# jamtrott/spmv-cache-trace

Hardware: AMD Instinct MI355X
Metric: spmv_csr_gflops (higher is better)
Workload: dtype f64

## Files before the change

### spmv-cache-trace_amd/csrc/csr_wavetile.hpp

```cpp
#pragma once

#include "tile_common.hpp"
#include "csr_blocktile.hpp"

namespace spmv {

constexpr int kShiftedMaxLen = 128;

#if defined(SPMV_HIP_EXPERIMENTS) && defined(SPMV_VI_ABLATE)
constexpr int kViAblate = SPMV_VI_ABLATE;
#else
constexpr int kViAblate = 0;
#endif
__device__ __forceinline__ int scalar_load_i32(const int32_t * p)
{
    typedef const int32_t __attribute__((address_space(4))) * const_ptr;
    return *reinterpret_cast<const_ptr>(reinterpret_cast<uintptr_t>(p));
}
}
#include "csr_stenciltile.hpp"
namespace spmv {

template <int QUADS, bool X32, bool VI = false>
__device__ __forceinline__ void tile_products_shifted(
// ... 378 lines not shown
    for (int p0 = 0; p0 < len; p0 += CH) {
#pragma unroll
        for (int i = 0; i < CH; ++i) {
            if (p0 + i < len) {
                const int c = scalar_load_i32(first_row + p0 + i) + first_row_base;
                xv[i] = X32 ? *reinterpret_cast<const v2d_a8 *>(reinterpret_cast<const char *>(x) + ((unsigned) (c + base) << 3))
                            : *reinterpret_cast<const v2d_a8 *>(x + c + base);
            }
        }
#pragma unroll
        for (int i = 0; i < CH; ++i) {
            if (p0 + i < len) {
                const int bi = lead + p0 + i;
                const int dw = scalar_load_i32(reinterpret_cast<const int32_t *>(vit) + (bi >> 2));
                const double val = vtab[(unsigned) (dw >> ((bi & 3) * 8)) & 0x7Fu];
                zA += val * xv[i].x;
                zB += val * xv[i].y;
            }
        }
    }
    if (both) {
        v2d_a8 out = {yv.x + zA, yv.y + zB};
        __builtin_nontemporal_store(out, reinterpret_cast<v2d_a8 *>(y + r0 + base));
        if (PEER) {
#pragma unroll
            for (int k = 0; k < kMaxPeers; ++k)
                if (k < peers.n) {
                    peers.y[k][r0 + base] = out.x;
                    peers.y[k][r0 + base + 1] = out.y;
                }
        }
    } else if (only_second) {
        y_store<PEER, true>(y, peers, r0 + base + 1, yv.y + zB);
    }
}

template <int LPR>
__device__ __forceinline__ double window_row_sum(const double * prod, int s, int e, int part)
{
    double z0 = 0.0, z1 = 0.0, z2 = 0.0, z3 = 0.0;
    int k = s + part;
    for (; k + 3 * LPR < e; k += 4 * LPR) {
        const double a = prod[k], b = prod[k + LPR], c = prod[k + 2 * LPR], d = prod[k + 3 * LPR];
        z0 += a;
        z1 += b;
        z2 += c;
        z3 += d;
    }
    for (; k < e; k += LPR)
        z0 += prod[k];
    return (z0 + z1) + (z2 + z3);
}

template <int TILE, int QUADS, bool C16, bool X32, bool VI, typename YStore>
__device__ __forceinline__ void tile_rows_multi_window(
    double * prod, const int32_t * __restrict__ p, const int32_t * __restrict__ j, const uint16_t * __restrict__ j16,
    const double * __restrict__ a, const double * __restrict__ x, const double * y_in, int r0, int k0, int k1, int nrows, int meta,
    int cbase, int cols, int lane, const uint8_t * __restrict__ vidx, ValueLookup vtab, YStore && store)
{
    const int kb = k0 & ~3;
    const int lanes_log2 = (meta >> kTileMetaLanesShift) & 0x7;
    const int sub = lane >> lanes_log2, part = lane & ((1 << lanes_log2) - 1);
    const int rowi = sub < nrows ? sub : nrows - 1;
    int ps, pe;
    if (meta & kTileMetaUniform) {
        ps = k0 + rowi * (meta & 0xFFFF);
// ... 6 lines not shown
    const bool narrow = C16 && (meta & kTileMetaNarrow);
    double z = 0.0;
    for (int base = kb; base < k1; base += TILE) {
        const int left = k1 - base;
        const int last = ((left < TILE ? left : TILE) - 1) & ~3;
        if (narrow)
            tile_products_narrow<QUADS, 0, VI>(prod, j16 + base, a + base, x + cbase, (unsigned) (cols - 1 - cbase), last, lane, vidx + base, vtab);
        else
            tile_products_wide<QUADS, X32, VI>(prod, j + base, a + base, x, last, lane, vidx + base, vtab);
        __builtin_amdgcn_fence(__ATOMIC_RELEASE, "wavefront");
        __builtin_amdgcn_wave_barrier();
        __builtin_amdgcn_fence(__ATOMIC_ACQUIRE, "wavefront");
        const int s = (ps > base ? ps : base) - base;
        const int e = (pe < base + TILE ? pe : base + TILE) - base;
        switch (lanes_log2) {
        case 3: z += window_row_sum<8>(prod, s, e, part); break;
        case 4: z += window_row_sum<16>(prod, s, e, part); break;
        default: z += window_row_sum<32>(prod, s, e, part); break;
        }
        __builtin_amdgcn_fence(__ATOMIC_RELEASE, "wavefront");
        __builtin_amdgcn_wave_barrier();
        __builtin_amdgcn_fence(__ATOMIC_ACQUIRE, "wavefront");
    }
    switch (lanes_log2) {
    case 3: z = group_sum<8>(z); break;
    case 4: z = group_sum<16>(z); break;
    case 5: z = group_sum<32>(z); break;
    default: z = group_sum<64>(z); break;
    }
    if (sub < nrows && part == 0)
        store(r0 + sub, yv + z);
}

template <int TILE, bool C16, bool X32, bool XCD, int ABL = 0, int XW = 0, bool PANELS = false, bool VI = false, bool PEER = false, bool LIST = false>
__global__ __launch_bounds__(256, (TILE <= 512 ? 8 : 4)) void csr_wavetile_kernel(
    int ntiles, const int4 * __restrict__ desc, const int32_t * __restrict__ p,
    const int32_t * __restrict__ j, const uint16_t * __restrict__ j16,
    const double * __restrict__ a, const double * __restrict__ x, const double * y_in_arg, double * y_arg,
    int nnz_total, int cols, int exact_order_and_nt, const int32_t * __restrict__ patterns, PanelInfo pinfo,
    const uint8_t * __restrict__ vidx = nullptr, const double * __restrict__ vtable = nullptr, int nvalues = 0,
    PeerY peers = PeerY{}, const int32_t * __restrict__ tile_list = nullptr)
{
    static_assert(!LIST || (!PANELS && !VI && !XCD), "the tile list is for the plain variants that follow a window kernel");
    static_assert(!PEER || !PANELS, "column panels add partial sums atomically: nothing to forward");
    constexpr int QUADS = TILE / 256;
    const int exact_order = exact_order_and_nt & 1;
    const bool nt_y = (exact_order_and_nt & 2) != 0;
    const int group_rows = (exact_order_and_nt >> 8) & 15;
    __shared__ __attribute__((aligned(16))) double prod_all[4][TILE + 4];
    __shared__ __attribute__((aligned(16))) uint32_t first_row_all[C16 ? 4 : 1][C16 ? kShiftedMaxLen : 1];
    __shared__ double vtab_lds[VI ? kMaxIndexedValues : 1];

    const int wave = __builtin_amdgcn_readfirstlane((int) threadIdx.x >> 6);
    const int lane = (int) __lane_id();
    int w;
    double * y = y_arg;
    const double * y_in = y_in_arg;
    if (PANELS) {
        const int pk = (int) blockIdx.x & 7;
        w = pinfo.first[pk] + ((int) blockIdx.x >> 3) * 4 + wave;
        if (w >= pinfo.first[pk + 1])
            return;
        y = y_arg - (size_t) pk * (size_t) pinfo.rows;
    } else {
        w = (XCD ? xcd_remap(blockIdx.x, (ntiles + 3) >> 2, true) : (int) blockIdx.x) * 4 + wave;
        if (!VI && w >= ntiles)
            return;
        if (LIST)
            w = __builtin_amdgcn_readfirstlane(tile_list[w]);
    }
    double * prod = prod_all[wave];
    static_assert(XW == 0 || TILE + 4 - XW >= 256 * (QUADS - 1), "the window may only overlap the last quad's product slots");
    double * xwin = prod + (XW ? TILE + 4 - XW : 0);

    const int wd = VI ? (w < ntiles ? w : ntiles - 1) : w;
    const TilePair dp = load_tile_pair(desc, wd);
    const int4 d0 = dp.d0, d1 = dp.d1;
    ValueLookup vtab{vtab_lds, false, 0.0, 0.0};
    if (VI) {
        vtab.tiny = nvalues <= 2;
        if (vtab.tiny) {
            vtab.t0 = vtable[0];
            vtab.t1 = vtable[1];
        } else {
            if (threadIdx.x < kMaxIndexedValues)
                vtab_lds[threadIdx.x] = vtable[threadIdx.x];
            __syncthreads();
        }
        if (w >= ntiles)
            return;
    }
    const int r0 = __builtin_amdgcn_readfirstlane(d0.x & ~kTileFlagPartial);
    const int partial = __builtin_amdgcn_readfirstlane(d0.x & kTileFlagPartial);
    const int k0 = __builtin_amdgcn_readfirstlane(d0.y);
    const int meta = __builtin_amdgcn_readfirstlane(d0.z);
    if (C16 && (meta & kTileMetaBlockWin))
        return;
    const int maxlen = meta & 0xFFFF;
    const int lanes_log2 = (meta >> kTileMetaLanesShift) & 0x7;
    const int cbase = __builtin_amdgcn_readfirstlane(d0.w);
    const int r1 = __builtin_amdgcn_readfirstlane(d1.x & ~kTileFlagPartial);
    const int k1 = __builtin_amdgcn_readfirstlane(d1.y);
    const int nrows = r1 - r0;
    const int kb = k0 & ~3;

    if (meta & kTileMetaFast) {
        if (VI && !kViAblate && C16 && TILE == 512 && !PANELS && (meta & kTileMetaValueRows) && (meta & kTileMetaShifted) && (meta & kTileMetaUniform)
            && (maxlen <= kLanePerRowMaxLen ? (lanes_log2 == 0 && nrows >= 2) : nrows >= kConstantRowMinRows)) {
            const bool pattern = (meta & kTileMetaPattern) != 0;
            tile_rows_pairs_constant<X32, PEER>(pattern ? patterns + (size_t) cbase * kPatStride + kPatRel : j + k0, pattern ? r0 : 0,
                                                vidx + kb, vtab, x, y_in, y, peers, r0, lane, maxlen, k0 - kb, nrows);
            return;
        }
        if (C16 && TILE == 512 && !PANELS && is_masked_stencil_tile(meta)) {
            const double * yin_t = y_in + r0;
            const double yA = yin_t[lane < nrows ? lane : nrows - 1];
            const double yB = yin_t[lane + kWave < nrows ? lane + kWave : nrows - 1];
            const int32_t * pat = patterns + (size_t) cbase * kPatStride;
            double zA, zB;
            tile_rows_masked_stencil<QUADS, X32, VI && !kViAblate>(prod, pat + kPatRel, __builtin_amdgcn_readfirstlane(pat[0]), j16 + k0, a + kb, vidx + kb,
                                                                   vtab, x, cols, r0, (k1 - 1 - kb) & ~3, lane, k0 - kb, nrows, zA, zB);
            if (lane < nrows)
                y_store<PEER, false>(y, peers, r0 + lane, yA + zA, nt_y);
            if (lane + kWave < nrows)
                y_store<PEER, false>(y, peers, r0 + lane + kWave, yB + zB, nt_y);
            return;
        }
        if (TILE == 512 && !PANELS && nrows > 1 && k1 - kb > TILE && lanes_log2 == 6) {
            const bool narrow = C16 && (meta & kTileMetaNarrow);
            tile_rows_long_registers<X32>(p, j, j16, narrow, a, x, narrow ? cbase : 0, (unsigned) (cols - 1 - (narrow ? cbase : 0)), y_in, r0, k0, k1,
                                          nrows, lane, [&](int idx, double v) { y_store<PEER, false>(y, peers, idx, v, nt_y); });
            return;
        }
        if (TILE == 512 && !PANELS && nrows > 1 && k1 - kb > TILE) {
            tile_rows_multi_window<TILE, QUADS, C16, X32, VI>(prod, p, j, j16, a, x, y_in, r0, k0, k1, nrows, meta, cbase, cols, lane, vidx, vtab,
                                                              [&](int idx, double v) { y_store<PEER, false>(y, peers, idx, v, nt_y); });
            return;
        }
// ... 199 lines not shown
```

### spmv-cache-trace_amd/csrc/internal.hpp

```cpp
#pragma once

#include "spmv_hip_plan.h"
#include "spmv_hip_symmetric.h"
#include "spmv_hip_multivec.h"
#include "spmv_hip_transpose.h"
#include "spmv_hip_f32values.h"
#include "spmv_hip_compact.h"
#include "spmv_hip_compact_f64.h"
#include "spmv_hip_compact_f32xy.h"
#include "spmv_hip_scaled.h"
#include "spmv_hip_dots.h"

#include <hip/hip_runtime.h>
#include <rccl/rccl.h>

#include <atomic>
#include <cstdint>
#include <string>
#include <vector>

#include "spmv_kernels.hpp"
#include "csr_segwin.hpp"

namespace spmvi {
// ... 93 lines not shown
    int split_rows = 0;
    bool balanced = false;
    int32_t * d_colh = nullptr;
    int32_t * d_hub_column = nullptr;
    double * d_hubx = nullptr;
    int nhubs = 0, hub_threshold = 0;
    long long hub_entries = 0;
    int multi_window_tiles = 0;
    int block_hint = 0;
    int block_offset = 0;
    bool block_skewed = false;
    int hints_tried = 0;
    bool hint_from_bits = false;
    int colshare_tiles = 0;
    long long colshare_entries = 0;
    int block_candidate = 0;
    const uint32_t * group_bits = nullptr;
    int block_cuts = 0;
    int break_rows = 0;
    int block_tiles = 0;
    long long block_entries = 0;
    int stencil_mask_tiles = 0;
    long long stencil_mask_entries = 0;
    int masked_block_tiles = 0;
    long long masked_block_entries = 0;
    size_t meta_bytes = 0;
    long long streamed_bytes = 0, shifted_entries = 0, narrow_entries = 0, uniform_rows = 0;
    uint8_t * d_vidx = nullptr;
    double * d_vtab = nullptr;
    int nvalues = 0;
    int value_row_tiles = 0;
    int4 * d_tiles_vi = nullptr;
    int ntiles_vi = 0;
    const double * values_from = nullptr;
    const double * values_wanted = nullptr;
    unsigned long long value_checksum = 0;
    mutable std::atomic<bool> verify_values_pending{false};
    unsigned long long column_checksum = 0;
    mutable std::atomic<bool> verify_pending{false};
};

struct spmv_hip_ctx {
    int device = 0;
    unsigned flags = 0;
    hipStream_t stream = nullptr;
    hipStream_t own_stream = nullptr;
    hipEvent_t ev0 = nullptr, ev1 = nullptr;
    bool timed = false;
    int format = 0;
    int32_t rows = 0, cols = 0, nnz = 0, row_length = 0, nnz2 = 0;
    int csr_algorithm = SPMV_HIP_CSR_AUTO;
    int csr_lanes = 0;
    spmv_hip_plan * plan = nullptr;
    spmv_hip_sym_plan * sym_plan = nullptr;
    spmv_hip_tr_plan * tr_plan = nullptr;
    spmv_hip_f32_plan * f32_plan = nullptr;
    float * d_val32 = nullptr;
    spmv_hip_c16_plan * c16_plan = nullptr;
    float *d_x32 = nullptr, *d_y32 = nullptr;
    double * d_dots = nullptr;
    size_t dots_work_bytes = 0;
    bool dots_run = false;
    spmv_hip_mv_plan * mv_plan = nullptr;
    double *d_bx = nullptr, *d_by = nullptr;
    int block_k = 0;
    bool block_x_set = false;
// ... 81 lines not shown
```

### spmv-cache-trace_amd/csrc/launch.hip

```cpp
#include "internal.hpp"
#ifdef SPMV_HIP_EXPERIMENTS
#include "csr_pipe.hpp"
#include <cstdlib>
#endif

#include <algorithm>

using namespace spmvi;

namespace {

template <bool DENSE, bool NT>
static auto run_kernel(bool yin_nt, bool yout_nt) -> decltype(&spmv::csr_runs_kernel<DENSE, NT, true, true>)
{
    return yin_nt ? (yout_nt ? spmv::csr_runs_kernel<DENSE, NT, true, true> : spmv::csr_runs_kernel<DENSE, NT, true, false>)
                  : (yout_nt ? spmv::csr_runs_kernel<DENSE, NT, false, true> : spmv::csr_runs_kernel<DENSE, NT, false, false>);
}

template <int LPR>
void launch_vector(const spmv_hip_plan * pl, const int32_t * p, const int32_t * j, const double * a,
                   const double * x, double * y, hipStream_t s)
{
    hipLaunchKernelGGL((spmv::csr_vector_kernel<LPR, kBlock>), dim3(pl->workgroups), dim3(kBlock), 0, s,
                       pl->rows, p, j, a, x, y);
// ... 248 lines not shown
                if (peers && pl->split_rows == 0 && !pl->d_blocks && !pl->d_segblocks) {
                    hipLaunchKernelGGL((spmv::csr_wavetile_kernel<512, true, true, false, 0, 256, false, false, true>), dim3(pl->workgroups), dim3(256), 0, s,
                                       pl->ntiles, pl->d_tiles, p, j, pl->d_col16, a, x, y_in, y, pl->nnz, pl->cols, exact, pl->d_patterns, spmv::PanelInfo{},
                                       (const uint8_t *) nullptr, (const double *) nullptr, 0, *peers);
                    *fused = 1;
                } else
                    hipLaunchKernelGGL((spmv::csr_wavetile_kernel<512, true, true, false, 0, 256>), dim3(pl->workgroups), dim3(256), 0, s,
                                       pl->ntiles, pl->d_tiles, p, j, pl->d_col16, a, x, y_in, y, pl->nnz, pl->cols, exact, pl->d_patterns, spmv::PanelInfo{});
            }
#ifdef SPMV_HIP_EXPERIMENTS
            else if (abl && c16 && x32 && pl->tile == 512) {
                if (abl == 1) hipLaunchKernelGGL((spmv::csr_wavetile_kernel<512, true, true, false, 1>), dim3(pl->workgroups), dim3(256), 0, s, pl->ntiles, pl->d_tiles, p, j, pl->d_col16, a, x, y_in, y, pl->nnz, pl->cols, exact, pl->d_patterns, spmv::PanelInfo{});
                else if (abl == 2) hipLaunchKernelGGL((spmv::csr_wavetile_kernel<512, true, true, false, 2>), dim3(pl->workgroups), dim3(256), 0, s, pl->ntiles, pl->d_tiles, p, j, pl->d_col16, a, x, y_in, y, pl->nnz, pl->cols, exact, pl->d_patterns, spmv::PanelInfo{});
                else hipLaunchKernelGGL((spmv::csr_wavetile_kernel<512, true, true, false, 3>), dim3(pl->workgroups), dim3(256), 0, s, pl->ntiles, pl->d_tiles, p, j, pl->d_col16, a, x, y_in, y, pl->nnz, pl->cols, exact, pl->d_patterns, spmv::PanelInfo{});
            }
#endif
            else if (pl->tile == 1024) {
                if (xcd) SPMV_WT_C(1024, true); else SPMV_WT_C(1024, false);
            } else if (peers && c16 && x32 && !xcd && pl->split_rows == 0 && !pl->d_blocks && !pl->d_segblocks) {
                if (pl->nvalues > 0 && pl->values_from == a)
                    hipLaunchKernelGGL((spmv::csr_wavetile_kernel<512, true, true, false, 0, 0, false, true, true>), dim3(vi_groups), dim3(256), 0, s,
                                       vi_ntiles, vi_tiles, p, j, pl->d_col16, a, x, y_in, y, pl->nnz, pl->cols, exact, pl->d_patterns,
                                       spmv::PanelInfo{}, pl->d_vidx, pl->d_vtab, pl->nvalues, *peers);
                else
                    hipLaunchKernelGGL((spmv::csr_wavetile_kernel<512, true, true, false, 0, 0, false, false, true>), dim3(pl->workgroups), dim3(256), 0, s,
                                       pl->ntiles, pl->d_tiles, p, j, pl->d_col16, a, x, y_in, y, pl->nnz, pl->cols, exact, pl->d_patterns,
                                       spmv::PanelInfo{}, (const uint8_t *) nullptr, (const double *) nullptr, 0, *peers);
                *fused = 1;
            } else if (c16 && x32 && pl->nvalues > 0 && pl->values_from == a) {
                if (xcd)
                    hipLaunchKernelGGL((spmv::csr_wavetile_kernel<512, true, true, true, 0, 0, false, true>), dim3(vi_groups), dim3(256), 0, s,
                                       vi_ntiles, vi_tiles, p, j, pl->d_col16, a, x, y_in, y, pl->nnz, pl->cols, exact, pl->d_patterns,
                                       spmv::PanelInfo{}, pl->d_vidx, pl->d_vtab, pl->nvalues);
                else
                    hipLaunchKernelGGL((spmv::csr_wavetile_kernel<512, true, true, false, 0, 0, false, true>), dim3(vi_groups), dim3(256), 0, s,
                                       vi_ntiles, vi_tiles, p, j, pl->d_col16, a, x, y_in, y, pl->nnz, pl->cols, exact, pl->d_patterns,
                                       spmv::PanelInfo{}, pl->d_vidx, pl->d_vtab, pl->nvalues);
            } else {
                if (xcd) SPMV_WT_C(512, true); else SPMV_WT_C(512, false);
            }
#undef SPMV_WT_C
#undef SPMV_WT_X
#undef SPMV_WT_LAUNCH
            if (c16 && pl->d_segblocks) {
                if (rest_forwards) {
                    if (pl->segwin_slots <= 2688)
                        hipLaunchKernelGGL((spmv::csr_segwin_kernel<512, 2688, true>), dim3(pl->nsegblocks), dim3(512), 0, s, pl->d_tiles,
                                           pl->d_segblocks, p, pl->d_col16, a, x, y_in, y, *peers);
                    else
                        hipLaunchKernelGGL((spmv::csr_segwin_kernel<512, 4096, true>), dim3(pl->nsegblocks), dim3(512), 0, s, pl->d_tiles,
                                           pl->d_segblocks, p, pl->d_col16, a, x, y_in, y, *peers);
                    *fused = 1;
                } else if (pl->segwin_slots <= 2688)
                    hipLaunchKernelGGL((spmv::csr_segwin_kernel<512, 2688>), dim3(pl->nsegblocks), dim3(512), 0, s, pl->d_tiles,
                                       pl->d_segblocks, p, pl->d_col16, a, x, y_in, y);
                else
                    hipLaunchKernelGGL((spmv::csr_segwin_kernel<512, 4096>), dim3(pl->nsegblocks), dim3(512), 0, s, pl->d_tiles,
                                       pl->d_segblocks, p, pl->d_col16, a, x, y_in, y);
            } else if (c16 && pl->d_blocks) {
#ifdef SPMV_HIP_EXPERIMENTS
                if (pl->flags & 0x2000u) {
                    hipLaunchKernelGGL((spmv::csr_blockwin_kernel<512>), dim3(pl->nblocks16), dim3(1024), 0, s, pl->ntiles,
                                       pl->d_tiles, pl->d_blocks, p, pl->d_col16, a, x, y_in, y);
                } else
#endif
                {
// ... 140 lines not shown
```

### spmv-cache-trace_amd/csrc/plan_csr.hip

```cpp
#include "internal.hpp"

#include <algorithm>
#include <cstdlib>
#include <cstring>
#include <new>
#include <system_error>
#include <thread>
#include <unordered_map>
#include <utility>

using namespace spmvi;

namespace {

constexpr size_t kStripedInts = (size_t) spmv::kCountStripes * spmv::kCountWidth;

template <typename T>
hipError_t read_striped(const T * d_counters, T * out, int n, hipStream_t s)
{
    T host[kStripedInts];
    hipError_t e = hipMemcpyAsync(host, d_counters, sizeof(host), hipMemcpyDeviceToHost, s);
    if (e == hipSuccess)
        e = hipStreamSynchronize(s);
    for (int i = 0; i < n; ++i) {
// ... 1870 lines not shown
    if (e == hipSuccess && rc == SPMV_HIP_OK) {
        rc = plan_csr_internal(&pl->inner, (int32_t) vrows, pl->cols, vrow_ptr.data(), SPMV_HIP_CSR_WAVETILE, 0,
                               (pl->flags | SPMV_HIP_FLAG_NO_X_WINDOW | SPMV_HIP_FLAG_NO_COLUMN_PANELS) & ~SPMV_HIP_FLAG_ROWS128, rows);
        if (rc == SPMV_HIP_OK)
            rc = spmv_hip_plan_csr_compress(pl->inner, pl->d_pcol, stream);
    }
    if (e != hipSuccess || rc != SPMV_HIP_OK) {
        if (pl->inner) { spmv_hip_plan_destroy(pl->inner); pl->inner = nullptr; }
        if (pl->d_vrow_ptr) { (void) hipFree(pl->d_vrow_ptr); pl->d_vrow_ptr = nullptr; }
        if (pl->d_pcol) { (void) hipFree(pl->d_pcol); pl->d_pcol = nullptr; }
        if (pl->d_pval) { (void) hipFree(pl->d_pval); pl->d_pval = nullptr; }
        return e != hipSuccess ? fail_hip(e, "column panels") : rc;
    }
    pl->pinfo = pl->inner->pinfo;
    int most = 0;
    for (int k = 0; k < 8; ++k)
        most = std::max(most, pl->pinfo.first[k + 1] - pl->pinfo.first[k]);
    pl->panel_blocks = (most + 3) / 4;
    pl->panels_from_col = d_column_index;
    pl->panels_from_val = d_value;
    pl->meta_bytes += (size_t) (vrows + 1) * sizeof(int32_t) + (size_t) pl->nnz * 12 + pl->inner->meta_bytes;
    {
        long long nonempty = 0;
        for (long long v = 0; v < vrows; ++v)
            nonempty += vrow_ptr[(size_t) v + 1] > vrow_ptr[(size_t) v];
        pl->streamed_bytes = pl->inner->streamed_bytes - 16LL * vrows + 16LL * nonempty;
        pl->shifted_entries = pl->inner->shifted_entries;
        pl->narrow_entries = pl->inner->narrow_entries;
        pl->uniform_rows = 0;
    }
    return SPMV_HIP_OK;
}

static hipError_t merge_constant_row_tiles(spmv_hip_plan * pl, const uint8_t * d_same_prev, hipStream_t s)
{
#if defined(SPMV_HIP_EXPERIMENTS) && defined(SPMV_VI_ABLATE)
    return hipSuccess;
#endif
    std::vector<int4> d((size_t) pl->ntiles + 1);
    hipError_t e = read_back(d.data(), pl->d_tiles, d.size() * sizeof(int4), s);
    if (e != hipSuccess)
        return e;
    std::vector<uint8_t> same_prev((size_t) pl->ntiles, 0);
    e = read_back(same_prev.data(), d_same_prev, same_prev.size(), s);
    if (e != hipSuccess)
        return e;
    std::vector<int32_t> pat;
    if (pl->d_patterns && pl->npatterns > 0) {
        pat.resize((size_t) pl->npatterns * spmv::kPatStride);
        e = read_back(pat.data(), pl->d_patterns, pat.size() * sizeof(int32_t), s);
        if (e != hipSuccess)
            return e;
    }
    const int want = spmv::kTileMetaValueRows | spmv::kTileMetaPattern | spmv::kTileMetaFast | spmv::kTileMetaUniform | spmv::kTileMetaShifted;
    auto mergeable = [&](int w) {
        return !(d[(size_t) w].x & spmv::kTileFlagPartial) && (d[(size_t) w].z & want) == want && d[(size_t) w].w >= 0
            && d[(size_t) w].w < pl->npatterns;
    };
    auto same_stencil = [&](int a, int b) {
        const int len = d[(size_t) a].z & 0xFFFF;
        if (len != (d[(size_t) b].z & 0xFFFF))
            return false;
        const int32_t * pa = pat.data() + (size_t) d[(size_t) a].w * spmv::kPatStride + spmv::kPatRel;
        const int32_t * pb = pat.data() + (size_t) d[(size_t) b].w * spmv::kPatStride + spmv::kPatRel;
        return d[(size_t) a].w == d[(size_t) b].w || std::equal(pa, pa + len, pb);
    };
    std::vector<int4> out;
    out.reserve(d.size());
    int merged_runs = 0;
    for (int w = 0; w < pl->ntiles;) {
        if (!mergeable(w)) {
            out.push_back(d[(size_t) w++]);
            continue;
        }
        int e_run = w + 1;
        while (e_run < pl->ntiles && mergeable(e_run) && same_stencil(w, e_run) && same_prev[(size_t) e_run])
            ++e_run;
        const int len = d[(size_t) w].z & 0xFFFF;
        const long long r_begin = d[(size_t) w].x, r_end = d[(size_t) e_run].x & 0x7FFFFFFF, k_begin = d[(size_t) w].y;
        if (e_run - w < 2 || (long long) d[(size_t) e_run].y - k_begin != (r_end - r_begin) * len) {
            for (; w < e_run; ++w)
                out.push_back(d[(size_t) w]);
            continue;
        }
        ++merged_runs;
        const long long run_rows = r_end - r_begin;
        const long long n = (run_rows + 127) / 128;
        if (len > spmv::kLanePerRowMaxLen && run_rows / n < spmv::kConstantRowMinRows) {
            --merged_runs;
            for (; w < e_run; ++w)
                out.push_back(d[(size_t) w]);
            continue;
        }
        long long r = r_begin;
        for (long long i = 0; i < n; ++i) {
            out.push_back(make_int4((int) r, (int) (k_begin + (r - r_begin) * len), d[(size_t) w].z, d[(size_t) w].w));
            r += run_rows / n + (i < run_rows % n ? 1 : 0);
        }
        w = e_run;
    }
    if (merged_runs == 0 || out.size() >= (size_t) pl->ntiles)
        return hipSuccess;
    const int n = (int) out.size();
    out.push_back(d[(size_t) pl->ntiles]);
    e = hipMalloc((void **) &pl->d_tiles_vi, out.size() * sizeof(int4));
    if (e == hipSuccess)
        e = hipMemcpy(pl->d_tiles_vi, out.data(), out.size() * sizeof(int4), hipMemcpyHostToDevice);
    if (e != hipSuccess) {
        if (pl->d_tiles_vi) (void) hipFree(pl->d_tiles_vi);
        pl->d_tiles_vi = nullptr;
        return e;
    }
    pl->ntiles_vi = n;
    return hipSuccess;
}

static void drop_value_dictionary(spmv_hip_plan * pl)
{
    if (pl->d_vidx) (void) hipFree(pl->d_vidx);
    if (pl->d_vtab) (void) hipFree(pl->d_vtab);
    if (pl->d_tiles_vi) (void) hipFree(pl->d_tiles_vi);
    pl->d_vidx = nullptr;
    pl->d_vtab = nullptr;
    pl->d_tiles_vi = nullptr;
    pl->ntiles_vi = 0;
    pl->nvalues = 0;
    pl->values_from = nullptr;
    pl->verify_values_pending = false;
}

int spmv_hip_plan_csr_index_values(spmv_hip_plan * pl, const double * d_value, void * stream)
{
    if (!pl)
        return fail(SPMV_HIP_ERR_INVALID, "plan is null");
    hipStream_t s = static_cast<hipStream_t>(stream);
    const size_t before = (pl->d_vidx ? (size_t) pl->nnz + 64 + spmv::kMaxIndexedValues * sizeof(double) : 0);
    drop_value_dictionary(pl);
    pl->values_wanted = d_value;
    pl->meta_bytes -= std::min(pl->meta_bytes, before);
    const bool other_variant = pl->inner || pl->d_blocks || pl->d_segblocks;
    if (pl->algorithm != SPMV_HIP_CSR_WAVETILE || pl->tile != 512 || pl->nnz == 0 || pl->ntiles == 0
        || (pl->balanced && (pl->flags & SPMV_HIP_FLAG_XCD_REMAP))
        || !pl->d_col16 || other_variant || pl->cols >= (1 << 29)
        || (pl->flags & SPMV_HIP_FLAG_NO_VALUE_INDEX))
        return (pl->inner || before == 0) ? SPMV_HIP_OK
                                          : plan_account(pl, pl->d_col16 != nullptr, s);
    if (!d_value)
        return fail(SPMV_HIP_ERR_INVALID, "null device pointer");
    unsigned long long * d_keys = nullptr;
    int * d_state = nullptr;
    std::vector<unsigned long long> keys((size_t) spmv::kDictSlots, spmv::kDictEmpty);
    int state[2] = {0, 0};
    hipError_t e = hipMalloc((void **) &d_keys, keys.size() * sizeof(unsigned long long));
    if (e == hipSuccess) e = hipMalloc((void **) &d_state, sizeof(state));
    if (e == hipSuccess) e = hipMemcpyAsync(d_keys, keys.data(), keys.size() * sizeof(unsigned long long), hipMemcpyHostToDevice, s);
    if (e == hipSuccess) e = hipMemsetAsync(d_state, 0, sizeof(state), s);
    if (e == hipSuccess && pl->nnz > 16384) {
        hipLaunchKernelGGL(spmv::value_dict_insert_kernel, dim3(1), dim3(256), 0, s, 8192LL, d_value, d_keys, d_state, spmv::kMaxIndexedValues);
// ... 22 lines not shown
        unsigned long long * d_table = nullptr;
        e = hipMalloc((void **) &d_table, (size_t) spmv::kMaxIndexedValues * sizeof(unsigned long long));
        if (e == hipSuccess) e = hipMalloc((void **) &pl->d_vtab, (size_t) spmv::kMaxIndexedValues * sizeof(double));
        if (e == hipSuccess) e = hipMalloc((void **) &pl->d_vidx, (size_t) pl->nnz + 64);
        if (e == hipSuccess) e = hipMemsetAsync(pl->d_vidx, 0, (size_t) pl->nnz + 64, s);
        if (e == hipSuccess) e = hipMemcpyAsync(d_table, table.data(), table.size() * sizeof(unsigned long long), hipMemcpyHostToDevice, s);
        if (e == hipSuccess) e = hipMemcpyAsync(pl->d_vtab, values.data(), values.size() * sizeof(double), hipMemcpyHostToDevice, s);
        if (e == hipSuccess) e = hipMemsetAsync(d_state, 0, sizeof(state), s);
        if (e == hipSuccess) {
            hipLaunchKernelGGL(spmv::value_index_kernel, dim3((unsigned) grid_for(pl->nnz, kBlock, cu_count() * 16)), dim3(256), 0, s,
                               (long long) pl->nnz, d_value, d_table, (int) table.size(), pl->d_vidx, d_state);
            e = hipGetLastError();
        }
        if (e == hipSuccess) e = hipMemcpyAsync(state, d_state, sizeof(state), hipMemcpyDeviceToHost, s);
        if (e == hipSuccess) e = hipStreamSynchronize(s);
        if (d_table) (void) hipFree(d_table);
        pl->value_row_tiles = 0;
        if (e == hipSuccess && state[1] == 0) {
            unsigned long long * d_count = nullptr;
            uint8_t * d_same_prev = nullptr;
            unsigned long long count[2] = {0, 0};
            e = hipMalloc((void **) &d_count, kStripedInts * sizeof(unsigned long long));
            if (e == hipSuccess) e = hipMalloc((void **) &d_same_prev, (size_t) pl->ntiles);
            if (e == hipSuccess) e = hipMemsetAsync(d_count, 0, kStripedInts * sizeof(unsigned long long), s);
            if (e == hipSuccess) {
                hipLaunchKernelGGL(spmv::value_rows_mark_kernel, dim3((unsigned) ((pl->ntiles + 3) / 4)), dim3(256), 0, s, pl->ntiles, pl->d_tiles,
                                   pl->d_vidx, spmv::kConstantRowMaxLen, d_count, d_same_prev);
                e = hipGetLastError();
            }
            if (e == hipSuccess) e = read_striped(d_count, count, 2, s);
            if (d_count) (void) hipFree(d_count);
            pl->value_row_tiles = (int) count[0];
            if (e == hipSuccess && count[0] > 0)
                e = merge_constant_row_tiles(pl, d_same_prev, s);
            if (d_same_prev) (void) hipFree(d_same_prev);
        }
        if (e == hipSuccess && state[1] == 0) {
            pl->nvalues = (int) table.size();
            pl->values_from = d_value;
            rc = device_value_checksum(d_value, pl->nnz, &pl->value_checksum, s);
            pl->verify_values_pending = true;
            pl->meta_bytes += (size_t) pl->nnz + 64 + spmv::kMaxIndexedValues * sizeof(double);
        } else {
            drop_value_dictionary(pl);
        }
    }
    if (d_keys) (void) hipFree(d_keys);
    if (d_state) (void) hipFree(d_state);
    if (e != hipSuccess) {
        drop_value_dictionary(pl);
        return fail_hip(e, "value dictionary");
    }
    if (rc != SPMV_HIP_OK) {
        drop_value_dictionary(pl);
        return rc;
    }
    if (pl->nvalues == 0 && before == 0)
        return SPMV_HIP_OK;
    return plan_account(pl, pl->d_col16 != nullptr, s);
}

int spmv_hip_plan_csr_refresh_values(spmv_hip_plan * pl, const int32_t * d_row_ptr, const int32_t * d_column_index,
                                     const double * d_value, void * stream)
{
    if (!pl)
        return fail(SPMV_HIP_ERR_INVALID, "plan is null");
    if (pl->nvalues > 0 || pl->d_vidx) {
        int rc = spmv_hip_plan_csr_index_values(pl, d_value, stream);
        if (rc != SPMV_HIP_OK)
            return rc;
    }
    if (!pl->inner)
        return SPMV_HIP_OK;
    if (!d_row_ptr || !d_column_index || !d_value)
        return fail(SPMV_HIP_ERR_INVALID, "null device pointer");
    if (d_column_index != pl->panels_from_col)
        return fail(SPMV_HIP_ERR_STATE, "the column panels were made from another column array");
    hipStream_t s = static_cast<hipStream_t>(stream);
    const unsigned grid = (unsigned) ((pl->rows + 255) / 256);
    hipLaunchKernelGGL(spmv::csr_panel_scatter_kernel, dim3(grid), dim3(256), 0, s, pl->rows, (pl->cols + 7) / 8, d_row_ptr,
                       d_column_index, d_value, pl->d_vrow_ptr, pl->d_pcol, pl->d_pval);
    HIP_TRY(hipGetLastError());
    pl->panels_from_val = d_value;
    return SPMV_HIP_OK;
}

int spmv_hip_plan_info(const spmv_hip_plan * pl, int64_t * out, int n)
{
    if (!pl || !out || n < 0)
        return fail(SPMV_HIP_ERR_INVALID, "plan/out null");
    const int64_t v[44] = {pl->algorithm, pl->lanes_per_row, pl->workgroups, pl->nblk,
                           pl->long_blocks, pl->rows, pl->nnz, (int64_t) pl->meta_bytes, pl->narrow_tiles,
                           pl->uniform_tiles, pl->shifted_tiles, pl->xwin_tiles, pl->blockwin_tiles,
                           pl->inner ? pl->inner->ntiles : 0, pl->streamed_bytes, pl->shifted_entries,
                           pl->narrow_entries, pl->uniform_rows, pl->inner ? 1 : 0, pl->balanced ? 1 : 0, pl->nvalues,
                           pl->segwin_tiles, pl->segwin_slots, pl->nvalues > 0 ? pl->value_row_tiles : 0,
                           pl->nvalues > 0 && pl->d_tiles_vi ? pl->ntiles_vi : 0, pl->nvalues > 0 ? 0 : pl->block_tiles,
                           pl->nvalues > 0 ? 0 : pl->block_entries, pl->nhubs, pl->hub_entries, pl->multi_window_tiles,
                           pl->ngroup_tiles, pl->nvalues > 0 ? 0 : pl->masked_block_tiles, pl->nvalues > 0 ? 0 : pl->masked_block_entries,
                           pl->stencil_mask_tiles, pl->stencil_mask_entries,
                           pl->nvalues > 0 ? 0 : pl->colshare_tiles, pl->nvalues > 0 ? 0 : pl->colshare_entries,
                           pl->colshare_tiles > 0 ? pl->block_hint : 0, pl->nrun_chunks, pl->run_tiles, pl->run_entries,
                           pl->run_masked_chunks, pl->nrun_chunks > 0 ? pl->nrun_rest : 0,
                           pl->nrun_chunks > 0 ? 1 + (pl->run_sweep ? 4 : 0) : 0};
    for (int i = 0; i < n && i < 44; ++i)
        out[i] = v[i];
    return SPMV_HIP_OK;
}

}
```

### spmv-cache-trace_amd/python/spmv_amd/capi.py

```python
import ctypes as C
import os

import numpy as np

PKG_ROOT = os.path.dirname(os.path.dirname(os.path.dirname(os.path.abspath(__file__))))
LIB_PATH = os.path.join(PKG_ROOT, "libspmv_hip.so")
EXPERIMENTS_LIB_PATH = os.path.join(PKG_ROOT, "libspmv_hip_experiments.so")
if os.environ.get("SPMV_HIP_EXPERIMENTS") == "1":
    LIB_PATH = EXPERIMENTS_LIB_PATH
elif os.environ.get("SPMV_HIP_EXPERIMENTS", "").endswith(".so"):
    LIB_PATH = os.path.abspath(os.environ["SPMV_HIP_EXPERIMENTS"])
HEADER_PATH = os.path.join(os.path.dirname(PKG_ROOT), "include", "spmv_hip.h")
HEADER_PATHS = [HEADER_PATH] + [os.path.join(os.path.dirname(PKG_ROOT), "include", n)
                                for n in ("spmv_hip_tuning.h", "spmv_hip_plan.h", "spmv_hip_symmetric.h", "spmv_hip_multivec.h",
                                          "spmv_hip_transpose.h", "spmv_hip_f32values.h", "spmv_hip_compact.h",
                                          "spmv_hip_compact_f64.h", "spmv_hip_compact_f32xy.h", "spmv_hip_scaled.h", "spmv_hip_dots.h",
                                          "spmv_hip_krylov.h", "spmv_hip_bicgstab.h", "spmv_hip_gmres.h", "spmv_hip_bjacobi.h",
                                          "spmv_hip_cheby.h", "spmv_hip_mcgs.h")]

OK = 0
ERR_INVALID, ERR_NO_DEVICE, ERR_HIP, ERR_ALLOC, ERR_STATE, ERR_OVERFLOW, ERR_ALIGN = -1, -2, -3, -4, -5, -6, -7
CSR_AUTO, CSR_SCALAR, CSR_VECTOR, CSR_ADAPTIVE, CSR_WAVETILE = 0, 1, 2, 3, 4
FLAG_XCD_REMAP, FLAG_EXACT_ORDER, FLAG_BIG_TILE, FLAG_NO_INDEX_COMPRESSION, FLAG_COO_KEEP_ORDER, FLAG_READ_ROW_PTR, FLAG_ROWS64, FLAG_ROWS128, FLAG_ELL_COLUMN_MAJOR = 0x1, 0x2, 0x8, 0x10, 0x20, 0x40, 0x80, 0x100, 0x200
FLAG_NO_SHIFTED_TILES = 0x400
# ... 451 lines not shown
        check(self.lib.spmv_hip_last_run_times(self.h, C.byref(k), C.byref(g)))
        return k.value, g.value

    def info(self):
        out = np.zeros(20, dtype=np.int64)
        check(self.lib.spmv_hip_ctx_info(self.h, out, 20))
        keys = ["format", "rows", "cols", "stored", "algorithm", "lanes_per_row", "workgroups",
                "row_blocks", "long_blocks", "device_bytes", "narrow_tiles", "shifted_tiles", "xwin_tiles",
                "blockwin_tiles", "panel_tiles", "streamed_bytes", "devices", "ell_path", "rccl_ranks", "pipelined"]
        return dict(zip(keys, out.tolist()))


class CsrPlan:

    def __init__(self, rows, cols, host_row_ptr, algorithm=CSR_AUTO, lanes_per_row=0, flags=0):
        self.lib = load()
        h = _vp()
        check(self.lib.spmv_hip_plan_csr(C.byref(h), rows, cols, _i32(host_row_ptr), algorithm,
                                         lanes_per_row, flags))
        self.h = h

    def close(self):
        if self.h:
            self.lib.spmv_hip_plan_destroy(self.h)
            self.h = None

    def __del__(self):
        try:
            self.close()
        except Exception:
            pass

    def info(self):
        out = np.zeros(44, dtype=np.int64)
        check(self.lib.spmv_hip_plan_info(self.h, out, 44))
        keys = ["algorithm", "lanes_per_row", "workgroups", "row_blocks", "long_blocks", "rows",
                "nnz", "meta_bytes", "narrow_tiles", "uniform_tiles", "shifted_tiles", "xwin_tiles", "blockwin_tiles", "panel_tiles",
                "streamed_bytes", "shifted_entries", "narrow_entries", "uniform_rows", "value_snapshot", "balanced", "indexed_values",
                "segwin_tiles", "segwin_slots", "value_row_tiles", "dictionary_launch_tiles", "block_tiles", "block_entries", "hub_columns", "hub_entries", "multi_window_tiles", "row_group_tiles",
                "masked_block_tiles", "masked_block_entries", "stencil_mask_tiles", "stencil_mask_entries",
                "group_tiles", "group_entries", "group_rows", "run_chunks", "run_tiles", "run_entries",
                "run_masked_chunks", "run_rest_tiles", "run_variant"]
        return dict(zip(keys, out.tolist()))

    def confirm_blocks(self, d_row_ptr, d_col, host_row_ptr=None, stream=0):
        hp = None if host_row_ptr is None else np.ascontiguousarray(host_row_ptr, dtype=np.int32)
        check(self.lib.spmv_hip_plan_csr_confirm_blocks(self.h, d_row_ptr, d_col, None if hp is None else hp.ctypes.data, stream))

    def compress(self, d_col, stream=0):
        check(self.lib.spmv_hip_plan_csr_compress(self.h, d_col, stream))

    def repack(self, d_row_ptr, d_col, d_val, stream=0):
        check(self.lib.spmv_hip_plan_csr_repack(self.h, d_row_ptr, d_col, d_val, stream))

    def spmv(self, d_row_ptr, d_col, d_val, d_x, d_y, stream=0):
        check(self.lib.spmv_hip_csr_spmv(self.h, d_row_ptr, d_col, d_val, d_x, d_y, stream))

    def spmv_out(self, d_row_ptr, d_col, d_val, d_x, d_y_in, d_y_out, stream=0):
        check(self.lib.spmv_hip_csr_spmv_out(self.h, d_row_ptr, d_col, d_val, d_x, d_y_in, d_y_out, stream))

    def verify(self, d_col, stream=0):
        check(self.lib.spmv_hip_plan_verify(self.h, d_col, stream))

    def index_values(self, d_val, stream=0):
        check(self.lib.spmv_hip_plan_csr_index_values(self.h, d_val, stream))

    def refresh_values(self, d_row_ptr, d_col, d_val, stream=0):
        check(self.lib.spmv_hip_plan_csr_refresh_values(self.h, d_row_ptr, d_col, d_val, stream))


def csr_triangle(rows, row_ptr, col):
    row_ptr, col = _i32(row_ptr), _i32(col)
    if len(row_ptr) < rows + 1:
        raise ValueError("row_ptr needs rows + 1 entries")
    if len(col) == 0:
# ... 627 lines not shown
```

Before: 1164.

## Bake dominant constant-value stencil into kernel arguments for value-indexed tiles

During planning, finds the most common (column offset pattern, coefficient) stencil among uniform value-indexed tiles, marks those tiles, and passes the stencil's offsets and coefficients as kernel arguments held in scalar registers. Marked tiles then skip loading column patterns, value indices and the value table and compute each row as a fixed stencil over x, two rows per lane. The plan also re-cuts constant-row runs on 128-row boundaries. This adds a planning pass with a device readback and a new kernel template instance with larger argument pressure, and it only pays off when the matrix has one stencil that dominates.

```diff
diff --git a/spmv-cache-trace_amd/csrc/csr_wavetile.hpp b/spmv-cache-trace_amd/csrc/csr_wavetile.hpp
--- a/spmv-cache-trace_amd/csrc/csr_wavetile.hpp
+++ b/spmv-cache-trace_amd/csrc/csr_wavetile.hpp
@@ -434,6 +434,67 @@
         }
     } else if (only_second) {
         y_store<PEER, true>(y, peers, r0 + base + 1, yv.y + zB);
+    }
+}
+
+constexpr int kDomMaxLen = 8;
+constexpr int kTileMetaDominant = 1 << 21;
+struct DomStencil {
+    int len;
+    int rel[kDomMaxLen];
+    double coef[kDomMaxLen];
+};
+
+template <int LEN, bool TWO>
+__device__ __forceinline__ void tile_rows_dominant(const DomStencil & dom, const double * __restrict__ x, const double * y_in,
+                                                   double * y, int r0, int lane, int nrows)
+{
+    constexpr int P = TWO ? 2 : 1;
+    const int top = nrows - 2;
+    int base[P];
+    v2d_a8 yv[P], xv[P][LEN];
+#pragma unroll
+    for (int q = 0; q < P; ++q)
+        base[q] = 128 * q + 2 * lane < top ? 128 * q + 2 * lane : top;
+#pragma unroll
+    for (int q = 0; q < P; ++q)
+        yv[q] = __builtin_nontemporal_load(reinterpret_cast<const v2d_a8 *>(y_in + r0 + base[q]));
+#pragma unroll
+    for (int q = 0; q < P; ++q)
+#pragma unroll
+        for (int p = 0; p < LEN; ++p)
+            xv[q][p] = *reinterpret_cast<const v2d_a8 *>(reinterpret_cast<const char *>(x) + ((unsigned) (r0 + dom.rel[p] + base[q]) << 3));
+#pragma unroll
+    for (int q = 0; q < P; ++q) {
+        double zA = 0.0, zB = 0.0;
+#pragma unroll
+        for (int p = 0; p < LEN; ++p) {
+            zA += dom.coef[p] * xv[q][p].x;
+            zB += dom.coef[p] * xv[q][p].y;
+        }
+        const int first = 128 * q + 2 * lane;
+        if (first <= top) {
+            const v2d_a8 out = {yv[q].x + zA, yv[q].y + zB};
+            __builtin_nontemporal_store(out, reinterpret_cast<v2d_a8 *>(y + r0 + base[q]));
+        } else if (first == nrows - 1) {
+            __builtin_nontemporal_store(yv[q].y + zB, y + r0 + base[q] + 1);
+        }
+    }
+}
+
+template <bool TWO>
+__device__ __forceinline__ void tile_rows_dominant_any(const DomStencil & dom, const double * __restrict__ x, const double * y_in,
+                                                       double * y, int r0, int lane, int nrows)
+{
+    switch (dom.len) {
+    case 1: tile_rows_dominant<1, TWO>(dom, x, y_in, y, r0, lane, nrows); break;
+    case 2: tile_rows_dominant<2, TWO>(dom, x, y_in, y, r0, lane, nrows); break;
+    case 3: tile_rows_dominant<3, TWO>(dom, x, y_in, y, r0, lane, nrows); break;
+    case 4: tile_rows_dominant<4, TWO>(dom, x, y_in, y, r0, lane, nrows); break;
+    case 5: tile_rows_dominant<5, TWO>(dom, x, y_in, y, r0, lane, nrows); break;
+    case 6: tile_rows_dominant<6, TWO>(dom, x, y_in, y, r0, lane, nrows); break;
+    case 7: tile_rows_dominant<7, TWO>(dom, x, y_in, y, r0, lane, nrows); break;
+    default: tile_rows_dominant<8, TWO>(dom, x, y_in, y, r0, lane, nrows); break;
     }
 }
 
@@ -506,16 +567,18 @@
         store(r0 + sub, yv + z);
 }
 
-template <int TILE, bool C16, bool X32, bool XCD, int ABL = 0, int XW = 0, bool PANELS = false, bool VI = false, bool PEER = false, bool LIST = false>
-__global__ __launch_bounds__(256, (TILE <= 512 ? 8 : 4)) void csr_wavetile_kernel(
+template <int TILE, bool C16, bool X32, bool XCD, int ABL = 0, int XW = 0, bool PANELS = false, bool VI = false, bool PEER = false, bool LIST = false,
+          int DOM = 0>
+__global__ __launch_bounds__(256, (TILE <= 512 ? (DOM == 2 ? 6 : 8) : 4)) void csr_wavetile_kernel(
     int ntiles, const int4 * __restrict__ desc, const int32_t * __restrict__ p,
     const int32_t * __restrict__ j, const uint16_t * __restrict__ j16,
     const double * __restrict__ a, const double * __restrict__ x, const double * y_in_arg, double * y_arg,
     int nnz_total, int cols, int exact_order_and_nt, const int32_t * __restrict__ patterns, PanelInfo pinfo,
     const uint8_t * __restrict__ vidx = nullptr, const double * __restrict__ vtable = nullptr, int nvalues = 0,
-    PeerY peers = PeerY{}, const int32_t * __restrict__ tile_list = nullptr)
+    PeerY peers = PeerY{}, const int32_t * __restrict__ tile_list = nullptr, DomStencil dom = DomStencil{})
 {
     static_assert(!LIST || (!PANELS && !VI && !XCD), "the tile list is for the plain variants that follow a window kernel");
+    static_assert(DOM == 0 || (VI && C16 && X32 && TILE == 512 && !XCD && !PANELS && !PEER && !LIST && ABL == 0 && XW == 0), "the dominant stencil belongs to the default dictionary launch");
     static_assert(!PEER || !PANELS, "column panels add partial sums atomically: nothing to forward");
     constexpr int QUADS = TILE / 256;
     const int exact_order = exact_order_and_nt & 1;
@@ -525,6 +588,10 @@
     __shared__ __attribute__((aligned(16))) uint32_t first_row_all[C16 ? 4 : 1][C16 ? kShiftedMaxLen : 1];
     __shared__ double vtab_lds[VI ? kMaxIndexedValues : 1];
 
+    if (DOM)
+        asm volatile("" ::"s"(x), "s"(y_in_arg), "s"(y_arg), "s"(dom.len), "s"(dom.rel[0]), "s"(dom.rel[1]), "s"(dom.rel[2]), "s"(dom.rel[3]),
+                     "s"(dom.rel[4]), "s"(dom.rel[5]), "s"(dom.rel[6]), "s"(dom.rel[7]), "s"(dom.coef[0]), "s"(dom.coef[1]), "s"(dom.coef[2]),
+                     "s"(dom.coef[3]), "s"(dom.coef[4]), "s"(dom.coef[5]), "s"(dom.coef[6]), "s"(dom.coef[7]));
     const int wave = __builtin_amdgcn_readfirstlane((int) threadIdx.x >> 6);
     const int lane = (int) __lane_id();
     int w;
@@ -578,6 +645,13 @@
     const int nrows = r1 - r0;
     const int kb = k0 & ~3;
 
+    if (DOM && (meta & kTileMetaDominant)) {
+        if (DOM == 2 && nrows > 128)
+            tile_rows_dominant_any<true>(dom, x, y_in, y, r0, lane, nrows);
+        else
+            tile_rows_dominant_any<false>(dom, x, y_in, y, r0, lane, nrows);
+        return;
+    }
     if (meta & kTileMetaFast) {
         if (VI && !kViAblate && C16 && TILE == 512 && !PANELS && (meta & kTileMetaValueRows) && (meta & kTileMetaShifted) && (meta & kTileMetaUniform)
             && (maxlen <= kLanePerRowMaxLen ? (lanes_log2 == 0 && nrows >= 2) : nrows >= kConstantRowMinRows)) {
diff --git a/spmv-cache-trace_amd/csrc/internal.hpp b/spmv-cache-trace_amd/csrc/internal.hpp
--- a/spmv-cache-trace_amd/csrc/internal.hpp
+++ b/spmv-cache-trace_amd/csrc/internal.hpp
@@ -149,6 +149,11 @@
     int value_row_tiles = 0;
     int4 * d_tiles_vi = nullptr;
     int ntiles_vi = 0;
+    bool vi_recut = false;
+    spmv::DomStencil dom_stencil{};
+    int dom_tiles = 0;
+    long long dom_rows = 0;
+    bool dom_two_pairs = false;
     const double * values_from = nullptr;
     const double * values_wanted = nullptr;
     unsigned long long value_checksum = 0;
diff --git a/spmv-cache-trace_amd/csrc/launch.hip b/spmv-cache-trace_amd/csrc/launch.hip
--- a/spmv-cache-trace_amd/csrc/launch.hip
+++ b/spmv-cache-trace_amd/csrc/launch.hip
@@ -304,6 +304,16 @@
                     hipLaunchKernelGGL((spmv::csr_wavetile_kernel<512, true, true, true, 0, 0, false, true>), dim3(vi_groups), dim3(256), 0, s,
                                        vi_ntiles, vi_tiles, p, j, pl->d_col16, a, x, y_in, y, pl->nnz, pl->cols, exact, pl->d_patterns,
                                        spmv::PanelInfo{}, pl->d_vidx, pl->d_vtab, pl->nvalues);
+#ifdef SPMV_HIP_EXPERIMENTS
+                else if (pl->d_tiles_vi && pl->dom_tiles > 0 && pl->dom_two_pairs)
+                    hipLaunchKernelGGL((spmv::csr_wavetile_kernel<512, true, true, false, 0, 0, false, true, false, false, 2>), dim3(vi_groups), dim3(256), 0, s,
+                                       vi_ntiles, vi_tiles, p, j, pl->d_col16, a, x, y_in, y, pl->nnz, pl->cols, exact, pl->d_patterns,
+                                       spmv::PanelInfo{}, pl->d_vidx, pl->d_vtab, pl->nvalues, spmv::PeerY{}, (const int32_t *) nullptr, pl->dom_stencil);
+#endif
+                else if (pl->d_tiles_vi && pl->dom_tiles > 0)
+                    hipLaunchKernelGGL((spmv::csr_wavetile_kernel<512, true, true, false, 0, 0, false, true, false, false, 1>), dim3(vi_groups), dim3(256), 0, s,
+                                       vi_ntiles, vi_tiles, p, j, pl->d_col16, a, x, y_in, y, pl->nnz, pl->cols, exact, pl->d_patterns,
+                                       spmv::PanelInfo{}, pl->d_vidx, pl->d_vtab, pl->nvalues, spmv::PeerY{}, (const int32_t *) nullptr, pl->dom_stencil);
                 else
                     hipLaunchKernelGGL((spmv::csr_wavetile_kernel<512, true, true, false, 0, 0, false, true>), dim3(vi_groups), dim3(256), 0, s,
                                        vi_ntiles, vi_tiles, p, j, pl->d_col16, a, x, y_in, y, pl->nnz, pl->cols, exact, pl->d_patterns,
diff --git a/spmv-cache-trace_amd/csrc/plan_csr.hip b/spmv-cache-trace_amd/csrc/plan_csr.hip
--- a/spmv-cache-trace_amd/csrc/plan_csr.hip
+++ b/spmv-cache-trace_amd/csrc/plan_csr.hip
@@ -1926,10 +1926,116 @@
     return SPMV_HIP_OK;
 }
 
-static hipError_t merge_constant_row_tiles(spmv_hip_plan * pl, const uint8_t * d_same_prev, hipStream_t s)
+static __global__ void first_row_bytes_kernel(int n, const int32_t * __restrict__ k, const uint8_t * __restrict__ vidx,
+                                              unsigned long long * __restrict__ out)
+{
+    const int i = (int) (blockIdx.x * blockDim.x + threadIdx.x);
+    if (i >= n)
+        return;
+    const uint8_t * b = vidx + k[i];
+    unsigned long long v = 0;
+    for (int q = 0; q < 8; ++q)
+        v |= (unsigned long long) b[q] << (8 * q);
+    out[i] = v;
+}
+
+static hipError_t mark_dominant_tiles(spmv_hip_plan * pl, std::vector<int4> & out, int n, const std::vector<int32_t> & pat,
+                                      const std::vector<double> & values, int max_rows, hipStream_t s)
+{
+    pl->dom_stencil = spmv::DomStencil{};
+    pl->dom_tiles = 0;
+    pl->dom_rows = 0;
+    const int want = spmv::kTileMetaValueRows | spmv::kTileMetaPattern | spmv::kTileMetaFast | spmv::kTileMetaUniform | spmv::kTileMetaShifted;
+    std::vector<int> cand;
+    std::vector<int32_t> first;
+    for (int w = 0; w < n; ++w) {
+        const int4 t = out[(size_t) w];
+        const int len = t.z & 0xFFFF, rows = (out[(size_t) w + 1].x & 0x7FFFFFFF) - (t.x & 0x7FFFFFFF);
+        if ((t.x & spmv::kTileFlagPartial) || (t.z & want) != want || (t.z & spmv::kTileMetaBlockWin) || ((t.z >> spmv::kTileMetaLanesShift) & 7) != 0
+            || len < 1 || len > spmv::kDomMaxLen || rows < 2 || rows > max_rows || t.w < 0 || t.w >= pl->npatterns
+            || (long long) out[(size_t) w + 1].y - t.y != (long long) rows * len)
+            continue;
+        cand.push_back(w);
+        first.push_back(t.y);
+    }
+    if (cand.empty())
+        return hipSuccess;
+    std::vector<unsigned long long> bytes(cand.size());
+    {
+        int32_t * d_first = nullptr;
+        unsigned long long * d_bytes = nullptr;
+        hipError_t e = hipMalloc((void **) &d_first, first.size() * sizeof(int32_t));
+        if (e == hipSuccess) e = hipMalloc((void **) &d_bytes, bytes.size() * sizeof(unsigned long long));
+        if (e == hipSuccess) e = hipMemcpyAsync(d_first, first.data(), first.size() * sizeof(int32_t), hipMemcpyHostToDevice, s);
+        if (e == hipSuccess) {
+            hipLaunchKernelGGL(first_row_bytes_kernel, dim3((unsigned) ((cand.size() + 255) / 256)), dim3(256), 0, s, (int) cand.size(), d_first,
+                               pl->d_vidx, d_bytes);
+            e = hipGetLastError();
+        }
+        if (e == hipSuccess) e = read_back(bytes.data(), d_bytes, bytes.size() * sizeof(unsigned long long), s);
+        if (d_first) (void) hipFree(d_first);
+        if (d_bytes) (void) hipFree(d_bytes);
+        if (e != hipSuccess)
+            return e;
+    }
+    struct Key {
+        int len;
+        int32_t rel[spmv::kDomMaxLen];
+        unsigned long long coef[spmv::kDomMaxLen];
+        bool operator==(const Key & o) const { return len == o.len && std::equal(rel, rel + len, o.rel) && std::equal(coef, coef + len, o.coef); }
+    };
+    auto key_of = [&](size_t i) {
+        const int4 t = out[(size_t) cand[i]];
+        Key k{};
+        k.len = t.z & 0xFFFF;
+        const int32_t * rel = pat.data() + (size_t) t.w * spmv::kPatStride + spmv::kPatRel;
+        for (int q = 0; q < k.len; ++q) {
+            k.rel[q] = rel[q];
+            std::memcpy(&k.coef[q], &values[(size_t) ((bytes[i] >> (8 * q)) & 0x7Fu)], sizeof(double));
+        }
+        return k;
+    };
+    std::vector<Key> keys;
+    std::vector<long long> rows_of;
+    std::vector<int> key_index(cand.size());
+    size_t hit = 0;
+    for (size_t i = 0; i < cand.size(); ++i) {
+        const Key k = key_of(i);
+        if (keys.empty() || !(keys[hit] == k)) {
+            for (hit = 0; hit < keys.size() && !(keys[hit] == k); ++hit) {}
+            if (hit == keys.size()) {
+                keys.push_back(k);
+                rows_of.push_back(0);
+            }
+        }
+        key_index[i] = (int) hit;
+        rows_of[hit] += (out[(size_t) cand[i] + 1].x & 0x7FFFFFFF) - (out[(size_t) cand[i]].x & 0x7FFFFFFF);
+    }
+    const size_t best = (size_t) (std::max_element(rows_of.begin(), rows_of.end()) - rows_of.begin());
+    pl->dom_stencil.len = keys[best].len;
+    for (int q = 0; q < keys[best].len; ++q) {
+        pl->dom_stencil.rel[q] = keys[best].rel[q];
+        std::memcpy(&pl->dom_stencil.coef[q], &keys[best].coef[q], sizeof(double));
+    }
+    for (size_t i = 0; i < cand.size(); ++i)
+        if (key_index[i] == (int) best) {
+            out[(size_t) cand[i]].z |= spmv::kTileMetaDominant;
+            ++pl->dom_tiles;
+        }
+    pl->dom_rows = rows_of[best];
+    return hipSuccess;
+}
+
+static hipError_t merge_constant_row_tiles(spmv_hip_plan * pl, const uint8_t * d_same_prev, const std::vector<double> & values, hipStream_t s)
 {
 #if defined(SPMV_HIP_EXPERIMENTS) && defined(SPMV_VI_ABLATE)
     return hipSuccess;
+#endif
+    bool mark = true, rows256 = false, aligned = true;
+#ifdef SPMV_HIP_EXPERIMENTS
+    if (const char * v = std::getenv("SPMV_HIP_VI_DOMINANT")) mark = std::atoi(v) != 0;
+    if (const char * v = std::getenv("SPMV_HIP_VI_ROWS256")) rows256 = std::atoi(v) != 0 && !(pl->flags & SPMV_HIP_FLAG_XCD_REMAP);
+    if (const char * v = std::getenv("SPMV_HIP_VI_ALIGN")) aligned = std::atoi(v) != 0;
 #endif
     std::vector<int4> d((size_t) pl->ntiles + 1);
     hipError_t e = read_back(d.data(), pl->d_tiles, d.size() * sizeof(int4), s);
@@ -1987,16 +2093,53 @@
             continue;
         }
         long long r = r_begin;
+        const long long head = std::min(r_end, (r_begin / 128 + 1) * 128) - r_begin, tail = r_end - (r_end - 1) / 128 * 128;
+        const long long n_aligned = (r_end - 1) / 128 - r_begin / 128 + 1;
+        if (aligned && len <= spmv::kLanePerRowMaxLen && n_aligned == n && head >= 2 && tail >= 2) {
+            while (r < r_end) {
+                out.push_back(make_int4((int) r, (int) (k_begin + (r - r_begin) * len), d[(size_t) w].z, d[(size_t) w].w));
+                r = std::min(r_end, (r / 128 + 1) * 128);
+            }
+            w = e_run;
+            continue;
+        }
         for (long long i = 0; i < n; ++i) {
             out.push_back(make_int4((int) r, (int) (k_begin + (r - r_begin) * len), d[(size_t) w].z, d[(size_t) w].w));
             r += run_rows / n + (i < run_rows % n ? 1 : 0);
         }
         w = e_run;
     }
-    if (merged_runs == 0 || out.size() >= (size_t) pl->ntiles)
+    const bool recut = merged_runs > 0 && out.size() < (size_t) pl->ntiles;
+    if (!recut)
+        out.assign(d.begin(), d.begin() + pl->ntiles);
+    int n = (int) out.size();
+    out.push_back(d[(size_t) pl->ntiles]);
+    if (mark) {
+        e = mark_dominant_tiles(pl, out, n, pat, values, 128, s);
+        if (e != hipSuccess)
+            return e;
+    }
+    if (!recut && pl->dom_tiles == 0)
         return hipSuccess;
-    const int n = (int) out.size();
-    out.push_back(d[(size_t) pl->ntiles]);
+    pl->vi_recut = recut;
+    if (rows256 && pl->dom_tiles > 0) {
+        std::vector<int4> two;
+        two.reserve(out.size());
+        for (int w = 0; w < n; ++w) {
+            two.push_back(out[(size_t) w]);
+            if (w + 1 < n && (out[(size_t) w].z & spmv::kTileMetaDominant) && (out[(size_t) w + 1].z & spmv::kTileMetaDominant)) {
+                const int ra = out[(size_t) w].x, rz = out[(size_t) w + 2].x & 0x7FFFFFFF;
+                if (rz - ra <= 256 && (!aligned || ra / 256 == (rz - 1) / 256)) {
+                    ++w;
+                    --pl->dom_tiles;
+                }
+            }
+        }
+        two.push_back(out[(size_t) n]);
+        n = (int) two.size() - 1;
+        out.swap(two);
+        pl->dom_two_pairs = true;
+    }
     e = hipMalloc((void **) &pl->d_tiles_vi, out.size() * sizeof(int4));
     if (e == hipSuccess)
         e = hipMemcpy(pl->d_tiles_vi, out.data(), out.size() * sizeof(int4), hipMemcpyHostToDevice);
@@ -2018,6 +2161,11 @@
     pl->d_vtab = nullptr;
     pl->d_tiles_vi = nullptr;
     pl->ntiles_vi = 0;
+    pl->vi_recut = false;
+    pl->dom_stencil = spmv::DomStencil{};
+    pl->dom_tiles = 0;
+    pl->dom_rows = 0;
+    pl->dom_two_pairs = false;
     pl->nvalues = 0;
     pl->values_from = nullptr;
     pl->verify_values_pending = false;
@@ -2106,7 +2254,7 @@
             if (d_count) (void) hipFree(d_count);
             pl->value_row_tiles = (int) count[0];
             if (e == hipSuccess && count[0] > 0)
-                e = merge_constant_row_tiles(pl, d_same_prev, s);
+                e = merge_constant_row_tiles(pl, d_same_prev, values, s);
             if (d_same_prev) (void) hipFree(d_same_prev);
         }
         if (e == hipSuccess && state[1] == 0) {
@@ -2163,21 +2311,23 @@
 {
     if (!pl || !out || n < 0)
         return fail(SPMV_HIP_ERR_INVALID, "plan/out null");
-    const int64_t v[44] = {pl->algorithm, pl->lanes_per_row, pl->workgroups, pl->nblk,
+    const bool dom = pl->nvalues > 0 && pl->d_tiles_vi && pl->dom_tiles > 0;
+    const int64_t v[47] = {pl->algorithm, pl->lanes_per_row, pl->workgroups, pl->nblk,
                            pl->long_blocks, pl->rows, pl->nnz, (int64_t) pl->meta_bytes, pl->narrow_tiles,
                            pl->uniform_tiles, pl->shifted_tiles, pl->xwin_tiles, pl->blockwin_tiles,
                            pl->inner ? pl->inner->ntiles : 0, pl->streamed_bytes, pl->shifted_entries,
                            pl->narrow_entries, pl->uniform_rows, pl->inner ? 1 : 0, pl->balanced ? 1 : 0, pl->nvalues,
                            pl->segwin_tiles, pl->segwin_slots, pl->nvalues > 0 ? pl->value_row_tiles : 0,
-                           pl->nvalues > 0 && pl->d_tiles_vi ? pl->ntiles_vi : 0, pl->nvalues > 0 ? 0 : pl->block_tiles,
+                           pl->nvalues > 0 && pl->d_tiles_vi && pl->vi_recut ? pl->ntiles_vi : 0, pl->nvalues > 0 ? 0 : pl->block_tiles,
                            pl->nvalues > 0 ? 0 : pl->block_entries, pl->nhubs, pl->hub_entries, pl->multi_window_tiles,
                            pl->ngroup_tiles, pl->nvalues > 0 ? 0 : pl->masked_block_tiles, pl->nvalues > 0 ? 0 : pl->masked_block_entries,
                            pl->stencil_mask_tiles, pl->stencil_mask_entries,
                            pl->nvalues > 0 ? 0 : pl->colshare_tiles, pl->nvalues > 0 ? 0 : pl->colshare_entries,
                            pl->colshare_tiles > 0 ? pl->block_hint : 0, pl->nrun_chunks, pl->run_tiles, pl->run_entries,
                            pl->run_masked_chunks, pl->nrun_chunks > 0 ? pl->nrun_rest : 0,
-                           pl->nrun_chunks > 0 ? 1 + (pl->run_sweep ? 4 : 0) : 0};
-    for (int i = 0; i < n && i < 44; ++i)
+                           pl->nrun_chunks > 0 ? 1 + (pl->run_sweep ? 4 : 0) : 0,
+                           dom ? pl->dom_tiles : 0, dom ? pl->dom_rows : 0, dom ? pl->dom_stencil.len : 0};
+    for (int i = 0; i < n && i < 47; ++i)
         out[i] = v[i];
     return SPMV_HIP_OK;
 }
diff --git a/spmv-cache-trace_amd/python/spmv_amd/capi.py b/spmv-cache-trace_amd/python/spmv_amd/capi.py
--- a/spmv-cache-trace_amd/python/spmv_amd/capi.py
+++ b/spmv-cache-trace_amd/python/spmv_amd/capi.py
@@ -507,15 +507,16 @@
             pass
 
     def info(self):
-        out = np.zeros(44, dtype=np.int64)
-        check(self.lib.spmv_hip_plan_info(self.h, out, 44))
+        out = np.zeros(47, dtype=np.int64)
+        check(self.lib.spmv_hip_plan_info(self.h, out, 47))
         keys = ["algorithm", "lanes_per_row", "workgroups", "row_blocks", "long_blocks", "rows",
                 "nnz", "meta_bytes", "narrow_tiles", "uniform_tiles", "shifted_tiles", "xwin_tiles", "blockwin_tiles", "panel_tiles",
                 "streamed_bytes", "shifted_entries", "narrow_entries", "uniform_rows", "value_snapshot", "balanced", "indexed_values",
                 "segwin_tiles", "segwin_slots", "value_row_tiles", "dictionary_launch_tiles", "block_tiles", "block_entries", "hub_columns", "hub_entries", "multi_window_tiles", "row_group_tiles",
                 "masked_block_tiles", "masked_block_entries", "stencil_mask_tiles", "stencil_mask_entries",
                 "group_tiles", "group_entries", "group_rows", "run_chunks", "run_tiles", "run_entries",
-                "run_masked_chunks", "run_rest_tiles", "run_variant"]
+                "run_masked_chunks", "run_rest_tiles", "run_variant",
+                "dominant_stencil_tiles", "dominant_stencil_rows", "dominant_stencil_length"]
         return dict(zip(keys, out.tolist()))
 
     def confirm_blocks(self, d_row_ptr, d_col, host_row_ptr=None, stream=0):
```

New measurement: 1162. No clear change (-0.2%).
